# jianwang-mpi/GlobalEgoMocap

Hardware: AMD Instinct MI355X
Metric: optimised windows/sec (10-frame, 15-joint) (higher is better)
Workload: dtype f32

## Files before the change

### globalegomocap_amd/csrc/energy_device.h

```cpp
#pragma once
#include "gem_internal.h"

namespace gem {

__device__ __forceinline__ double wave_sum(double v) { return wave_sum_dpp(v); }
typedef float f32x4_t __attribute__((ext_vector_type(4)));

constexpr int MAXT = 16;
constexpr int MAXJ = GEM_MAX_JOINTS;
constexpr int ENERGY_SCRATCH = MAXT * MAXJ * 3;

template <bool BLOCK_SYNC>
__device__ __forceinline__ void energy_sync() {
    if (BLOCK_SYNC) {
        __syncthreads();
    } else {
        __builtin_amdgcn_fence(__ATOMIC_RELEASE, "workgroup");
        __builtin_amdgcn_wave_barrier();
        __builtin_amdgcn_fence(__ATOMIC_ACQUIRE, "workgroup");
    }
}

template <int NE, int NP>
struct EnergyPre {
    float x0[NE];
    float mb[NP];
    int par[NP];
    int key[NP];
    f32x4_t val[NP];
};
struct NoEnergyPre {};

template <int NT, int CN, typename F>
__device__ __forceinline__ void lane_pass(int lane, int n, F f) {
    if constexpr (CN > 0) {
#pragma unroll
        for (int it = 0; it < (CN + NT - 1) / NT; ++it) {
            const int e = lane + it * NT;
            if (e < CN) f(e, it);
        }
    } else {
        int it = 0;
        for (int e = lane; e < n; e += NT, ++it) f(e, it);
    }
}

template <int CT, int CJ>
__device__ __forceinline__ void energy_prefetch(const EnergyArgs& a, int b, int lane, EnergyPre<(CT * CJ * 3 + 63) / 64, (CT * CJ + 63) / 64>& pre) {
    constexpr int n = CT * CJ * 3, TJ = CT * CJ;
#pragma unroll
    for (int it = 0; it < (n + 63) / 64; ++it) {
        const int e = lane + it * 64;
        pre.x0[it] = e < n ? a.X0[(size_t)b * n + e] : 0.f;
    }
#pragma unroll
    for (int it = 0; it < (TJ + 63) / 64; ++it) {
        const int p = lane + it * 64;
        pre.mb[it] = 0.f; pre.par[it] = 0; pre.key[it] = -1; pre.val[it] = f32x4_t{0.f, 0.f, 0.f, 0.f};
        if (p < TJ) {
            const int j = p % CJ;
            pre.mb[it] = a.mean_bone[(size_t)b * CJ + j];
            pre.par[it] = a.parents[j];
            if (a.tex_key && a.wr != 0.f) {
                const size_t ci = (size_t)b * TJ + p;
                pre.key[it] = a.tex_key[ci];
                pre.val[it] = *reinterpret_cast<const f32x4_t*>(a.tex_val + ci * 4);
            }
        }
    }
}

struct FisheyeUV { float zz, nn, inv, rho, drho, ux, uy, u, v; };
__device__ __forceinline__ FisheyeUV fisheye_uv(const float* poly, int n_poly, float cx, float cy, float x, float y, float z) {
    FisheyeUV q;
    q.zz = -z;
    q.nn = sqrtf(x * x + y * y);
    q.inv = 1.f / q.nn;
    const float theta = atanf(q.zz / q.nn);
    float rho = poly[0], drho = 0.f, ti = 1.f;
    for (int i = 1; i < n_poly; ++i) {
        drho += (float)i * poly[i] * ti;
        ti *= theta;
        rho += ti * poly[i];
    }
    q.rho = rho; q.drho = drho;
    q.ux = x * q.inv; q.uy = y * q.inv;
    q.u = q.ux * rho + cx; q.v = q.uy * rho + cy;
    return q;
}

struct HeatTap { float fx, fy; bool in, xl, xr, yt, yb; int xa, xb, ya, yc; };
__device__ __forceinline__ HeatTap heat_tap(float u, float v, int H, int W) {
    HeatTap k;
    const float gxn = ((u - 128.f) - 512.f) / 512.f, gyn = (v - 512.f) / 512.f;
    const float ix = ((gxn + 1.f) / 2.f) * (float)(W - 1);
    const float iy = ((gyn + 1.f) / 2.f) * (float)(H - 1);
    const float fx0 = floorf(ix), fy0 = floorf(iy);
    k.fx = ix - fx0; k.fy = iy - fy0;
    k.in = fx0 >= -1.f && fx0 < (float)W && fy0 >= -1.f && fy0 < (float)H;
    const int x0i = k.in ? (int)fx0 : 0, y0i = k.in ? (int)fy0 : 0;
    k.xl = k.in && x0i >= 0; k.xr = k.in && x0i + 1 < W; k.yt = y0i >= 0; k.yb = y0i + 1 < H;
    k.xa = x0i < 0 ? 0 : x0i; k.xb = x0i + 1 < W ? x0i + 1 : W - 1;
    k.ya = y0i < 0 ? 0 : y0i; k.yc = y0i + 1 < H ? y0i + 1 : H - 1;
    return k;
}

__device__ __forceinline__ float heat_bilinear(const HeatTap& k, float& nw, float& ne, float& sw, float& se) {
    nw = (k.yt && k.xl) ? nw : 0.f;
    ne = (k.yt && k.xr) ? ne : 0.f;
    sw = (k.yb && k.xl) ? sw : 0.f;
    se = (k.yb && k.xr) ? se : 0.f;
    const float gxw = 1.f - k.fx, gyw = 1.f - k.fy;
    return nw * gxw * gyw + ne * k.fx * gyw + sw * gxw * k.fy + se * k.fx * k.fy;
}

template <bool BLOCK_SYNC, int NT = 64, int CT = 0, int CJ = 0, bool XS_IS_SRC = false, typename Pre = NoEnergyPre>
__device__ __forceinline__ void energy_window(const EnergyArgs& a, int b, int lane, const float* xsrc, int ldx, float* xs,
                                              float* gs, float* bs, float* as, float* gdst, int ldg, int gcols,
                                              uint16_t* gdst_b = nullptr, const float* x0_w = nullptr, const float* mb_w = nullptr,
                                              const int* par_w = nullptr, const int* ch_w = nullptr, const Pre* pre = nullptr) {
    static_assert(NT == 64 || BLOCK_SYNC, "more than one wavefront per window needs workgroup barriers");
    static_assert((CT > 0) == (CJ > 0), "give both compile-time dimensions or none");
    constexpr bool HAS_PRE = !__is_same(Pre, NoEnergyPre);
    static_assert(!HAS_PRE || (NT == 64 && CT > 0), "prefetched inputs are per lane of ONE wavefront with compile-time dimensions");
    const int T = CT ? CT : a.T, J = CJ ? CJ : a.J, JC = J * 3, n = T * JC;
    constexpr int CN = CT * CJ * 3, CP = CT * CJ;
    const float* x0 = x0_w ? x0_w : a.X0 + (size_t)b * n;
    const float* mbone = mb_w ? mb_w : a.mean_bone + (size_t)b * J;
    const int* parents = par_w ? par_w : a.parents;
    const int* children = ch_w ? ch_w : a.children;

    double e3d = 0, esm = 0, ebone = 0, evae = 0, erep = 0;
    lane_pass<NT, CN>(lane, n, [&](int e, int it) {
        const int t = e / JC, c = e - t * JC;
        const float x = xsrc[t * ldx + c];
        if (!XS_IS_SRC) xs[e] = x;
        float x0v;
        if constexpr (HAS_PRE) x0v = pre->x0[it]; else x0v = x0[e];
        const float d = x - x0v;
        e3d += (double)(d * d);
        evae += (double)(x * x);
        gs[e] = 2.f * a.w3d * d + 2.f * a.wv * x;
    });
    energy_sync<BLOCK_SYNC>();
    lane_pass<NT, CN>(lane, n, [&](int e, int) {
        const int t = e / JC;
        float acc = 0.f;
        if (t >= 1 && t <= T - 2) {
            acc = xs[e - JC] - 2.f * xs[e] + xs[e + JC];
            esm += (double)(acc * acc);
        }
        as[e] = acc;
    });
    lane_pass<NT, CP>(lane, T * J, [&](int p, int it) {
        const int t = p / J, j = p - t * J;
        int par;
        float mbv;
        if constexpr (HAS_PRE) { par = pre->par[it]; mbv = pre->mb[it]; } else { par = parents[j]; mbv = mbone[j]; }
        const float* xj = xs + (t * J + j) * 3;
        const float* xp = xs + (t * J + par) * 3;
        const float bx = xj[0] - xp[0], by = xj[1] - xp[1], bz = xj[2] - xp[2];
        const float len = sqrtf(bx * bx + by * by + bz * bz);
        const float diff = len - mbv;
        ebone += (double)(diff * diff);
        const float coef = len > 0.f ? 2.f * a.wb * diff / len : 0.f;
        float* o = bs + (t * J + j) * 3;
        o[0] = coef * bx; o[1] = coef * by; o[2] = coef * bz;
    });
    energy_sync<BLOCK_SYNC>();
    lane_pass<NT, CN>(lane, n, [&](int e, int) {
        const int t = e / JC;
        float g = gs[e];
        const float w2 = 2.f * a.ws;
        if (t >= 1 && t <= T - 2) g -= 2.f * w2 * as[e];
        if (t >= 2) g += w2 * as[e - JC];
        if (t <= T - 3) g += w2 * as[e + JC];
        gs[e] = g;
    });
    energy_sync<BLOCK_SYNC>();
    lane_pass<NT, CP>(lane, T * J, [&](int p, int it) {
        const int t = p / J, j = p - t * J;
        float gx = bs[p * 3 + 0], gy = bs[p * 3 + 1], gz = bs[p * 3 + 2];
        const int* ch = children + j * MAXJ;
        for (int q = 0; q < MAXJ && ch[q] >= 0; ++q) {
            const float* o = bs + (t * J + ch[q]) * 3;
            gx -= o[0]; gy -= o[1]; gz -= o[2];
        }
        if (a.wr != 0.f) {
            const float x = xs[p * 3 + 0], y = xs[p * 3 + 1], z = xs[p * 3 + 2];
            const FisheyeUV q = fisheye_uv(a.poly, a.n_poly, a.cx, a.cy, x, y, z);
            const float zz = q.zz, nn = q.nn, inv = q.inv, rho = q.rho, drho = q.drho, ux = q.ux, uy = q.uy;
            if (nn == 0.f) erep = __builtin_nan("");
            const HeatTap k = heat_tap(q.u, q.v, a.H, a.W);
            const float fx = k.fx, fy = k.fy;
            const bool in = k.in;
            const int xa = k.xa, xb = k.xb, ya = k.ya, yc = k.yc;
            const float* hm = a.heat + ((size_t)(a.frame0[b] + t) * a.H * a.W) * J + j;
            float nw, ne, sw, se;
            const int key = in ? (ya * a.W + xa) | ((yc * a.W + xb) << 16) : -1;
            const size_t ci = (size_t)b * (T * J) + p;
            bool hit = false;
            if (a.tex_key && in) {
                if constexpr (HAS_PRE) {
                    hit = pre->key[it] == key;
                    if (hit) { nw = pre->val[it][0]; ne = pre->val[it][1]; sw = pre->val[it][2]; se = pre->val[it][3]; }
                } else {
                    hit = a.tex_key[ci] == key;
                    if (hit) {
                        const f32x4_t c = *reinterpret_cast<const f32x4_t*>(a.tex_val + ci * 4);
                        nw = c[0]; ne = c[1]; sw = c[2]; se = c[3];
                    }
                }
            }
            if (!hit) {
                nw = hm[((size_t)ya * a.W + xa) * J];
                ne = hm[((size_t)ya * a.W + xb) * J];
                sw = hm[((size_t)yc * a.W + xa) * J];
                se = hm[((size_t)yc * a.W + xb) * J];
                if (a.tex_key && in) {
                    a.tex_key[ci] = key;
                    *reinterpret_cast<f32x4_t*>(a.tex_val + ci * 4) = f32x4_t{nw, ne, sw, se};
                }
            }
            const float val = heat_bilinear(k, nw, ne, sw, se);
            const float gxw = 1.f - fx, gyw = 1.f - fy;
            erep -= (double)val;
            const float dix = (ne - nw) * gyw + (se - sw) * fy;
            const float diy = (sw - nw) * gxw + (se - ne) * fx;
            const float gu = -a.wr * dix * ((float)(a.W - 1) / 1024.f);
            const float gv = -a.wr * diy * ((float)(a.H - 1) / 1024.f);
            const float r2 = nn * nn + zz * zz;
            const float dth_dn = -zz / r2, dth_dz = -nn / r2;
            const float i3 = inv * inv * inv;
            const float dudx = rho * (inv - x * x * i3) + ux * drho * dth_dn * ux;
            const float dudy = rho * (-x * y * i3) + ux * drho * dth_dn * uy;
            const float dudz = ux * drho * dth_dz;
            const float dvdx = rho * (-x * y * i3) + uy * drho * dth_dn * ux;
            const float dvdy = rho * (inv - y * y * i3) + uy * drho * dth_dn * uy;
            const float dvdz = uy * drho * dth_dz;
            gx += gu * dudx + gv * dvdx;
            gy += gu * dudy + gv * dvdy;
            gz += gu * dudz + gv * dvdz;
        }
        gs[p * 3 + 0] += gx; gs[p * 3 + 1] += gy; gs[p * 3 + 2] += gz;
    });
    energy_sync<BLOCK_SYNC>();
    if (CT > 0 && gcols == 64) {
        lane_pass<NT, CT * 64>(lane, T * 64, [&](int i, int) {
            const int t = i >> 6, c = i & 63;
            const float v = c < JC ? gs[t * JC + c] : 0.f;
            if (gdst_b) gdst_b[t * ldg + c] = (uint16_t)(__builtin_bit_cast(unsigned int, (float)(__bf16)v) >> 16);
            else gdst[t * ldg + c] = v;
        });
    } else {
        for (int i = lane; i < T * gcols; i += NT) {
            const int t = i / gcols, c = i - t * gcols;
            const float v = c < JC ? gs[t * JC + c] : 0.f;
            if (gdst_b) gdst_b[t * ldg + c] = (uint16_t)(__builtin_bit_cast(unsigned int, (float)(__bf16)v) >> 16);
            else gdst[t * ldg + c] = v;
        }
    }
    e3d = wave_sum(e3d); esm = wave_sum(esm); ebone = wave_sum(ebone); evae = wave_sum(evae); erep = wave_sum(erep);
    if (NT > 64) {
        double* red = reinterpret_cast<double*>(as);
        const int wv = lane >> 6;
        if ((lane & 63) == 0) { red[wv * 5 + 0] = e3d; red[wv * 5 + 1] = esm; red[wv * 5 + 2] = ebone; red[wv * 5 + 3] = evae; red[wv * 5 + 4] = erep; }
        __syncthreads();
        if (lane == 0) {
            e3d = esm = ebone = evae = erep = 0.0;
            for (int w = 0; w < NT / 64; ++w) {
                e3d += red[w * 5 + 0]; esm += red[w * 5 + 1]; ebone += red[w * 5 + 2]; evae += red[w * 5 + 3]; erep += red[w * 5 + 4];
            }
        }
    }
    if (lane == 0) {
        if (a.parts) {
            double* p = a.parts + (size_t)b * 5;
            p[0] = e3d; p[1] = esm; p[2] = ebone; p[3] = evae; p[4] = erep;
        }
        a.f[b] = a.dw3d * e3d + a.dws * esm + a.dwb * ebone + a.dwv * evae + a.dwr * erep;
    }
}

}
```

### globalegomocap_amd/csrc/gem_internal.h

```cpp
#pragma once
#if defined(__HIP_DEVICE_COMPILE__) && !defined(GEM_NO_PACKED_FP32)
#error "compile with: -Xclang -target-feature -Xclang -packed-fp32-ops -DGEM_NO_PACKED_FP32 (__graft_entry__.NO_PACKED_FP32)"
#endif

#include <hip/hip_runtime.h>
#include <stdint.h>
#include <atomic>
#include <set>
#include <string>
#include <vector>

#include "../../include/gem_hip.h"

namespace gem {

constexpr int PAD = 64;
constexpr float LEAKY_SLOPE = 0.01f;
constexpr double BN_EPS = 1e-5;
constexpr int MAX_HIST = 128;
constexpr int MAXJ_ERR = GEM_MAX_JOINTS;
constexpr int N_LOG = 1 << 16;
constexpr int TRACE_ROUNDS = 64;

inline int pad64(int x) { return (x + PAD - 1) / PAD * PAD; }
// ... 263 lines not shown
    if (s.dyn_W > 0) {
        const DynSplit d = dyn_split(*s.m_dev, 64, s.CT, s.dyn_W, s.n_tiles, s.ldc);
        nslab = d.SK;
        stride = d.slab;
    }
}
bool rows_can_fuse_compaction(const gem_handle* h, const Layer& L, int lda, int ldc, int B, bool slabs);
int launch_splitk_reduce(gem_handle* h, int epi, int nslab, size_t slab, const float* bias, const float* aux, float* C, int M, int N,
                         int ldc, const int* m_dev, hipStream_t s, int dyn_W = 0, int n_tiles = 0);
int launch_gemm_bf16(gem_handle* h, const Layer& L, int epi, int nprod, const float* A, int lda, const float* aux, float* Cout,
                     int ldc, int M, int T, hipStream_t s, const GemmOpts& o);

enum Narrow {
    NARROW_BATCHED = 0,
    NARROW_TAIL_F32 = 1,
    NARROW_TAIL_BF16 = 2
};
struct Route {
    int precision = 0;
    Narrow narrow = NARROW_BATCHED;
    bool front = false;
    int tail_wgs = 0;
    int tail_cap = 0;
    Repack repack = REPACK_KERNEL;
};
enum Call { CALL_DECODE = 0, CALL_EVALUATE = 1, CALL_ROUNDS = 2 };
Route plan_route(const gem_handle* h, int stage, int B, Call call);

struct EnergyArgs;
int evaluate_bf16(gem_handle* h, const Route& rt, int stage, int B, const EnergyArgs& ea, hipStream_t s, bool forward_only, const RoundSet* rs,
                  SlabSrc* grad);
int gemm_bf16a(gem_handle* h, const Layer& L, int epi, const uint16_t* A, int lda, const uint16_t* aux, void* C, bool out_bf16,
               int ldc, int M, hipStream_t s, int family, bool allow_split, const GemmOpts& o = GemmOpts());
int make_layer_images(std::vector<void*>& owner, Layer* L, int taps, int N, int K, const float* w, const float* bias);
int launch_f32_to_bf16(const float* src, uint16_t* dst, size_t n, hipStream_t s);
int launch_f32_split_bf16(const float* src, uint16_t* hi, uint16_t* lo, size_t n, hipStream_t s);

int launch_pack_pose(const float* src, float* dst, int rows, int C, hipStream_t s);
int launch_unpack_pose(const float* src, float* dst, int rows, int C, hipStream_t s);
int launch_reparam(const float* mulv, const float* eps, float* mu, float* logvar, float* z, float* z2, int B, int D, int Dp,
                   hipStream_t s);
int launch_pad_latent(const float* z, float* zp, int B, int D, int Dp, hipStream_t s);
int launch_unpad_latent(const float* zp, float* z, int B, int D, int Dp, hipStream_t s);

struct EnergyArgs {
    const float* Xp;
    const float* X0;
    const float* heat;
    const int32_t* frame0;
    const float* mean_bone;
    float* dXp;
    uint16_t* dXp_b;
    double* f;
    double* parts;
    float w3d, ws, wb, wv, wr;
    double dw3d, dws, dwb, dwv, dwr;
    int T, J, H, W, n_poly;
    float poly[GEM_MAX_POLY];
    float cx, cy;
    const int* parents;
    const int* children;
    int* tex_key;
    float* tex_val;
    const int* n_dev;
    const int* perm;
};
int launch_energy(gem_handle* h, const EnergyArgs& a, int B, hipStream_t s);

constexpr int TAIL_MAX_LAYERS = 6;
struct TailLayerDev { const float* w4; const float* bias; int K, N; };
struct TailArgs {
    int n, B, G, forward_only, escr, mask_first;
    int waves, rows;
    int maxnt;
    SlabSrc in_slab;
    const float* in_bias;
    int in_bias_ld;
    long long* dbg_ts;
    TailLayerDev fwd[TAIL_MAX_LAYERS], bwd[TAIL_MAX_LAYERS];
    const float* a_in;
    float* g_out;
    uint16_t* g_out_b;
    float* Xp;
    int off_act[TAIL_MAX_LAYERS + 1], ld_act[TAIL_MAX_LAYERS + 1], off_g[2], ld_g, off_red, off_escr, off_zero, off_pre;
    EnergyArgs e;
};
size_t plan_tail(const std::vector<Layer>& dec, int start, int T, int J, TailArgs* out, bool shared = false);
void fill_tail_args(const gem_handle* h, const StageNet& net, const Route& rt, int B, bool forward_only, const SlabSrc& in_slab,
                    const EnergyArgs& ea, const RoundSet* rs, TailArgs* ta);
size_t plan_tail_for(const gem_handle* h, const std::vector<Layer>& dec, int start, int wgs, TailArgs* out);

constexpr int TB_MAX_LAYERS = 6;
struct TailB16Layer { int K, N; const float* bias; };
struct TailB16Args {
    int n, B, G, nrt, forward_only, mask_first;
    SlabSrc in_slab;
    const float* in_bias;
    int in_bias_ld;
    const uint16_t* a_in_b;
    uint16_t* g_out_b;
    float* Xp;
    long long* dbg_ts;
    const uint16_t* wstream;
    int steps_f, steps_total;
    TailB16Layer fwd[TB_MAX_LAYERS], bwd[TB_MAX_LAYERS];
    int off_act[TB_MAX_LAYERS + 1], ld_act[TB_MAX_LAYERS + 1];
    int off_mask[TB_MAX_LAYERS], ld_mask[TB_MAX_LAYERS];
    int off_x, escr, off_mb, off_zero, off_tab;
    int off_bwin, off_epair;
    EnergyArgs e;
};
size_t plan_tail_bf16(const std::vector<Layer>& dec, int start, int T, int J, TailB16Args* out, int nrt = 5);
int tail_bf16_row_tiles(const gem_handle* h, int B, int T);
int build_tail_bf16_stream(gem_handle* h, StageNet& net);
int launch_tail_bf16(gem_handle* h, const TailB16Args& a, size_t lds_bytes, hipStream_t s, const RoundSet* rs = nullptr);
int launch_tail(gem_handle* h, const TailArgs& a, size_t lds_bytes, hipStream_t s, const RoundSet* rs = nullptr);
int tail_cap_workgroups(const gem_handle* h, const std::vector<Layer>& dec, int start);
int launch_mean_bone(gem_handle* h, const float* pose, int n_frames, float* out, hipStream_t s);
int launch_gather_windows(const float* frames, const int32_t* frame0, float* out, int B, int T, int JC, hipStream_t s);
int launch_relative_global(const float* local, const double* cams, const int32_t* frame0, float* rel, int B, int T, int J,
                           hipStream_t s);
int launch_to_global(const float* rel, const double* cams, const int32_t* frame0, double* out, int B, int T, int J,
                     hipStream_t s);

int launch_errors(gem_handle* h, const double* est, const double* mid, const double* opt, const double* gt, int F,
                  const double* bone_mm, double* frame_out, double* out, hipStream_t s, int n_seq);
int launch_merge(const double* win, double* tmp, double* out, int n_chunks, int wpc, int T, int JC, int overlap, int smooth,
                 hipStream_t s);
size_t errors_frame_lds_bytes(int J);
void drop_graphs(gem_handle* h);
int post_scratch(gem_handle* h, size_t elems);
int launch_lift(gem_handle* h, const float* heat, const double* depth, int F, const double* poly, int n_poly, int up, int pad_x,
                int pad_y, double* out64, float* out32, hipStream_t s);

int launch_lbfgs_init(gem_handle* h, int B, hipStream_t s);
int launch_lbfgs_advance(gem_handle* h, int B, const gem_lbfgs_opts& o, const RoundSet& rs, const SlabSrc& grad, hipStream_t s);
int launch_lbfgs_stats(gem_handle* h, int B, gem_window_stats* out, hipStream_t s);
int launch_compact(gem_handle* h, const RoundSet& rs, int B, int force_all, hipStream_t s, int zero_after = 0);
int launch_lbfgs_debug_read(gem_handle* h, int B, gem_lbfgs_debug_state* out, float* x, float* d, float* trial, hipStream_t s);


}
```

### globalegomocap_amd/csrc/tail.hip

```cpp
#include <algorithm>

#include "energy_device.h"

namespace gem {

typedef float f32x16 __attribute__((ext_vector_type(16)));
typedef float f32x4 __attribute__((ext_vector_type(4)));

__device__ __forceinline__ float bf16_round(float x) {
    const __bf16 b = (__bf16)x;
    return (float)b;
}

constexpr int TAIL_WAVES = 8;
constexpr int TAIL_THREADS = TAIL_WAVES * 64;
constexpr int TAIL_WAVES_SHARED = 4;

constexpr int TAIL_ROWS = 16;

#ifndef TAIL_PREFETCH_BLOCKS
#define TAIL_PREFETCH_BLOCKS 1
#endif
#ifndef TAIL_RING_DEPTH
#define TAIL_RING_DEPTH 2
#endif
#ifndef TAIL_PREFETCH_EARLY
#define TAIL_PREFETCH_EARLY 1
#endif
template <int W, int MAXNT>
struct TailSched {
    static constexpr bool DEEP = W == TAIL_WAVES && MAXNT <= 2;
    static constexpr int P = DEEP ? TAIL_PREFETCH_BLOCKS : 1;
    static constexpr int D = DEEP ? TAIL_RING_DEPTH : 2;
    static constexpr int NTP = DEEP ? MAXNT : 1;
    static constexpr int PW = P < D - 1 ? P : D - 1;
    static constexpr bool EARLY = DEEP && TAIL_PREFETCH_EARLY;
    static_assert(P >= 1 && D >= 2 && D <= 4, "ring of two to four register sets");
};
template <int W, int MAXNT>
struct TailPre {
    f32x4 b[TailSched<W, MAXNT>::P][4];
    f32x4 bx[TailSched<W, MAXNT>::NTP > 1 ? TailSched<W, MAXNT>::NTP - 1 : 1][TailSched<W, MAXNT>::PW][4];
    float bias[TailSched<W, MAXNT>::NTP];
};

template <int W, int MAXNT>
__device__ __forceinline__ void tail_prefetch(const TailLayerDev L, TailPre<W, MAXNT>& dst) {
    using S = TailSched<W, MAXNT>;
    const int lane = threadIdx.x & 63, wave = __builtin_amdgcn_readfirstlane(threadIdx.x >> 6);
    const int c = lane & 15, q = lane >> 4;
    const int n0 = wave * 16;
    if (n0 >= L.N) return;
    const int nblk = 3 * (L.K / 64);
    const int nb = nblk <= S::P ? nblk : S::PW;
    const char* p = reinterpret_cast<const char*>(reinterpret_cast<const f32x4*>(L.w4) + n0);
    const unsigned vo = (unsigned)(q * L.N + c) * 16u;
#pragma unroll
    for (int i = 0; i < S::NTP; ++i) {
        if (n0 + 16 * W * i < L.N) {
#pragma unroll
            for (int s = 0; s < (i == 0 ? S::P : S::PW); ++s) {
                if (s < nb) {
#pragma unroll
                    for (int g = 0; g < 4; ++g) {
                        const f32x4 v = *reinterpret_cast<const f32x4*>(p + (((size_t)16 * s + 4 * g) * L.N + 16 * W * i) * 16 + vo);
                        if (i == 0) dst.b[s][g] = v;
                        else dst.bx[i > 0 ? i - 1 : 0][s][g] = v;
                    }
                }
            }
            if constexpr (S::DEEP) dst.bias[i] = L.bias ? L.bias[n0 + 16 * W * i + c] : 0.f;
        }
    }
}

template <int W, int MAXNT, int NT, typename Epi>
__device__ __forceinline__ void tail_gemm_nt(const float* in, int ld_in, const float* zero_line, const TailLayerDev L,
                                             const TailLayerDev next, bool has_next, int T, int R, TailPre<W, MAXNT>& pre, Epi epi,
                                             int c0 = 0, bool use_pre = true) {
    using S = TailSched<W, MAXNT>;
    constexpr int P = S::P, D = S::D, NTP = S::NTP, PW = S::PW;
    const int tid = threadIdx.x, lane = tid & 63, wave = __builtin_amdgcn_readfirstlane(tid >> 6);
    const int fr = lane & 15, fq = lane >> 4;
// ... 67 lines not shown
        if (use_pre) {
#pragma unroll
            for (int s = 0; s < P; ++s) {
                if (s < PW || whole) {
#pragma unroll
                    for (int g = 0; g < 4; ++g) asm volatile("" : "+v"(pre.b[s][g]));
                }
            }
#pragma unroll
            for (int i = 1; i < (NT < NTP ? NT : NTP); ++i)
#pragma unroll
                for (int s = 0; s < PW; ++s)
#pragma unroll
                    for (int g = 0; g < 4; ++g) asm volatile("" : "+v"(pre.bx[i - 1][s][g]));
        }
        if (has_next) tail_prefetch<W, MAXNT>(next, pre_next);
    }
    TAIL_LOAD_A(0, a[0]);
    if (whole) {
        if constexpr (P >= 3 && NT == 1) {
            static_assert(P == 3, "a layer has at least three blocks: K = 64, three taps");
#pragma unroll
            for (int t = 0; t < P; ++t) TAIL_STEP(t, t, false, (&pre.b[t]));
        }
    } else {
#pragma unroll
        for (int s = 0; s < D - 1; ++s)
#pragma unroll
            for (int i = 0; i < NT; ++i) {
                if (s < PW && i < NTP && use_pre) {
#pragma unroll
                    for (int g = 0; g < 4; ++g) b[s][i][g] = i == 0 ? pre.b[s][g] : pre.bx[i > 0 ? i - 1 : 0][s < PW ? s : 0][g];
                } else TAIL_LOAD_B1(s, b[s], i);
            }
        const int nl = nblk - (D - 1), ngrp = nl / D, r = nl - ngrp * D;
        for (int grp = 0; grp < ngrp; ++grp) {
#pragma unroll
            for (int j = 0; j < D; ++j) TAIL_STEP(grp * D + j, j, true, b[j]);
        }
        const int blk0 = ngrp * D;
#pragma unroll
        for (int rr = 0; rr < D; ++rr) {
            if (r != rr) continue;
#pragma unroll
            for (int t = 0; t < rr + D - 1; ++t) TAIL_STEP(blk0 + t, t, t < rr, b[t % D]);
        }
    }
    if constexpr (S::EARLY) pre = pre_next;
    else if (has_next) tail_prefetch<W, MAXNT>(next, pre);
#undef TAIL_STEP
#undef TAIL_INTERLEAVE
#undef TAIL_LOAD_A
#undef TAIL_LOAD_B
#undef TAIL_LOAD_B1
#undef TAIL_COMPUTE
#pragma unroll
    for (int i = 0; i < NT; ++i) epi(acc[i], 4 * fq, n0 + TS * i + fr, bv[i]);
}

template <int W, int MAXNT, typename Epi>
__device__ __forceinline__ void tail_gemm(const float* in, int ld_in, const float* zero_line, const TailLayerDev L,
                                          const TailLayerDev next, bool has_next, int T, int R, TailPre<W, MAXNT>& pre, Epi epi) {
    if constexpr (W == TAIL_WAVES_SHARED) {
        if (L.N > 32 * W) {
            tail_gemm_nt<W, MAXNT, 2>(in, ld_in, zero_line, L, next, false, T, R, pre, epi);
            tail_gemm_nt<W, MAXNT, 2>(in, ld_in, zero_line, L, next, has_next, T, R, pre, epi, 32 * W, false);
        } else if (L.N > 16 * W) tail_gemm_nt<W, MAXNT, 2>(in, ld_in, zero_line, L, next, has_next, T, R, pre, epi);
        else tail_gemm_nt<W, MAXNT, 1>(in, ld_in, zero_line, L, next, has_next, T, R, pre, epi);
    } else {
        if constexpr (MAXNT >= 4) {
            if (L.N > 32 * W) { tail_gemm_nt<W, MAXNT, 4>(in, ld_in, zero_line, L, next, has_next, T, R, pre, epi); return; }
        }
        if (L.N > 16 * W) tail_gemm_nt<W, MAXNT, 2>(in, ld_in, zero_line, L, next, has_next, T, R, pre, epi);
        else tail_gemm_nt<W, MAXNT, 1>(in, ld_in, zero_line, L, next, has_next, T, R, pre, epi);
    }
}

template <int MAXNT>
struct TailTiles {
template <int NL, int W>
static __global__ __launch_bounds__(64 * W, W == TAIL_WAVES_SHARED ? 3 : 2) void decoder_tail_kernel(TailArgs a) {
    constexpr int THREADS = 64 * W;
    constexpr bool TIGHT = W == TAIL_WAVES_SHARED;
    constexpr int STAGE_U = 2048 / THREADS;
    constexpr int PRE_E = TAIL_THREADS / THREADS;
    extern __shared__ __attribute__((aligned(16))) float lds[];
    const int tid = threadIdx.x, lane = tid & 63, wave = __builtin_amdgcn_readfirstlane(tid >> 6);
    const int T = a.e.T;
    int probe = 0;
#define TAIL_PROBE()                                                                                   \
    if (a.dbg_ts && blockIdx.x == 0 && tid == 0) {                                                     \
        a.dbg_ts[2 * probe] = clock64();                                                               \
        a.dbg_ts[2 * probe + 1] = wall_clock64();                                                      \
        ++probe;                                                                                       \
    }
    const int w0 = blockIdx.x * a.G;
    const int B = a.e.n_dev ? *a.e.n_dev : a.B;
    if (w0 >= B) return;
    const int nwin = min(a.G, B - w0);
    const int R = nwin * T;
    const size_t row0 = (size_t)w0 * T;

    {
        const int K0 = a.fwd[0].K, q4 = K0 / 4, n4 = (TIGHT ? a.rows : TAIL_ROWS) * q4;
        float* dst = lds + a.off_act[0];
        if (a.in_slab.base) {
            int nslab;
            size_t stride;
            slab_layout(a.in_slab, nslab, stride);
            for (int u = 0; u < STAGE_U; ++u) {
                const int i = tid + u * THREADS, r = i / q4, c = (i - r * q4) * 4;
                if (i >= n4) break;
                f32x4 v = {0.f, 0.f, 0.f, 0.f};
                if (r < R) {
                    const float* p = a.in_slab.base + (row0 + r) * K0 + c;
                    for (int z0 = 0; z0 < nslab; z0 += 8) {
                        f32x4 t[8];
#pragma unroll
                        for (int k = 0; k < 8; ++k) t[k] = *reinterpret_cast<const f32x4*>(p + (size_t)min(z0 + k, nslab - 1) * stride);
#pragma unroll
                        for (int k = 0; k < 8; ++k)
                            if (z0 + k < nslab) v += t[k];
                    }
                    v += *reinterpret_cast<const f32x4*>(a.in_bias + (r % T) * a.in_bias_ld + c);
#pragma unroll
                    for (int q = 0; q < 4; ++q) v[q] = v[q] > 0.f ? v[q] : v[q] * LEAKY_SLOPE;
                }
                *reinterpret_cast<f32x4*>(dst + r * a.ld_act[0] + c) = v;
            }
        } else {
            f32x4 v[STAGE_U];
#pragma unroll
            for (int u = 0; u < STAGE_U; ++u) {
                const int i = tid + u * THREADS, r = i / q4, c = (i - r * q4) * 4;
                v[u] = f32x4{0.f, 0.f, 0.f, 0.f};
                if (i < n4 && r < R) v[u] = *reinterpret_cast<const f32x4*>(a.a_in + (row0 + r) * K0 + c);
            }
#pragma unroll
            for (int u = 0; u < STAGE_U; ++u) {
                const int i = tid + u * THREADS, r = i / q4, c = (i - r * q4) * 4;
                if (i < n4) *reinterpret_cast<f32x4*>(dst + r * a.ld_act[0] + c) = v[u];
            }
        }
        if (tid < 64) lds[a.off_zero + tid] = 0.f;
    }
    float pre_x0[PRE_E], pre_mb = 0.f;
    int pre_par = 0, pre_ch[PRE_E];
#pragma unroll
    for (int k = 0; k < PRE_E; ++k) { pre_x0[k] = 0.f; pre_ch[k] = -1; }
    static_assert(MAXJ * MAXJ <= TAIL_THREADS && MAXJ <= 64, "the children table is parked by PRE_E passes of the workgroup");
    const bool pre_on = a.G == 1 && !a.forward_only && T * a.e.J * 3 <= TAIL_THREADS;
    if (pre_on) {
        const int J = a.e.J, n = T * J * 3, bw = a.e.perm ? a.e.perm[w0] : w0;
#pragma unroll
        for (int k = 0; k < PRE_E; ++k) {
            const int e = tid + k * THREADS;
            if (e < n) pre_x0[k] = a.e.X0[(size_t)bw * n + e];
            if (e < J * MAXJ) pre_ch[k] = a.e.children[e];
        }
        if (tid < J) { pre_mb = a.e.mean_bone[(size_t)bw * J + tid]; pre_par = a.e.parents[tid]; }
    }
    TAIL_PROBE();
    __syncthreads();
    TAIL_PROBE();

    TailPre<W, MAXNT> bpre;
    tail_prefetch<W, MAXNT>(a.fwd[0], bpre);
#pragma unroll
    for (int i = 0; i < NL; ++i) {
        const bool last = (i + 1 == NL);
        float* out = lds + a.off_act[i + 1];
        const int ldo = a.ld_act[i + 1];
        float* Xp = last ? a.Xp : nullptr;
        const TailLayerDev nxt = !last ? a.fwd[i + 1 < NL ? i + 1 : i] : a.bwd[NL - 1];
        tail_gemm<W, MAXNT>(lds + a.off_act[i], a.ld_act[i], lds + a.off_zero, a.fwd[i], nxt, !last || !a.forward_only, T, R, bpre,
                  [&](const f32x4& acc, int r0, int col, float bv) {
#pragma unroll
                      for (int e = 0; e < 4; ++e) {
                          float v = acc[e] + bv;
                          if (!last) v = v > 0.f ? v : v * LEAKY_SLOPE;
                          if (!TIGHT || r0 + e < a.rows) out[(r0 + e) * ldo + col] = v;
                          if (Xp && r0 + e < R) Xp[(row0 + r0 + e) * PAD + col] = v;
                      }
                  });
        if (i == 0 && pre_on) {
            const int J = a.e.J, n = T * J * 3;
            float* pre = lds + a.off_pre;
            int* prei = reinterpret_cast<int*>(pre + n + J);
#pragma unroll
            for (int k = 0; k < PRE_E; ++k) {
                const int e = tid + k * THREADS;
                if (e < n) pre[e] = pre_x0[k];
                if (e < J * MAXJ) prei[J + e] = pre_ch[k];
            }
            if (tid < J) { pre[n + tid] = pre_mb; prei[tid] = pre_par; }
        }
        __syncthreads();
        TAIL_PROBE();
    }
    if (a.forward_only) return;

    float* g_cur = lds + a.off_g[0];
    float* g_nxt = lds + a.off_g[1];
    if (a.G == 1) {
        float* scr = lds + a.off_escr;
        const int J = a.e.J, n = T * J * 3;
        const float* pre = lds + a.off_pre;
        const int* prei = reinterpret_cast<const int*>(pre + n + J);
        if (T == 10 && J == 15)
            energy_window<true, THREADS, 10, 15>(a.e, a.e.perm ? a.e.perm[w0] : w0, tid, lds + a.off_act[NL], a.ld_act[NL], scr,
                                                      scr + a.escr, scr + 2 * a.escr, scr + 3 * a.escr, g_cur, a.ld_g, a.fwd[NL - 1].N,
                                                      nullptr, pre_on ? pre : nullptr, pre_on ? pre + n : nullptr, pre_on ? prei : nullptr,
                                                      pre_on ? prei + J : nullptr);
        else
            energy_window<true, THREADS>(a.e, a.e.perm ? a.e.perm[w0] : w0, tid, lds + a.off_act[NL], a.ld_act[NL], scr,
                                              scr + a.escr, scr + 2 * a.escr, scr + 3 * a.escr, g_cur, a.ld_g, a.fwd[NL - 1].N,
                                              nullptr, pre_on ? pre : nullptr, pre_on ? pre + n : nullptr, pre_on ? prei : nullptr,
                                              pre_on ? prei + J : nullptr);
    } else if (wave < nwin) {
        float* scr = lds + a.off_escr + wave * 4 * a.escr;
        energy_window<false>(a.e, a.e.perm ? a.e.perm[w0 + wave] : w0 + wave, lane,
                             lds + a.off_act[NL] + wave * T * a.ld_act[NL], a.ld_act[NL], scr, scr + a.escr,
                             scr + 2 * a.escr, scr + 3 * a.escr, g_cur + wave * T * a.ld_g, a.ld_g, a.fwd[NL - 1].N);
    }
    __syncthreads();
    TAIL_PROBE();

#pragma unroll
    for (int i = NL - 1; i >= 0; --i) {
        const float* act = lds + a.off_act[i];
        const int lda = a.ld_act[i];
        const int ldg = a.ld_g;
        float* gout = a.g_out;
        uint16_t* gout_b = a.g_out_b;
        const int K0 = a.fwd[0].K;
        tail_gemm<W, MAXNT>(g_cur, a.ld_g, lds + a.off_zero, a.bwd[i], a.bwd[i > 0 ? i - 1 : 0], i > 0, T, R, bpre,
                  [&](const f32x4& acc, int r0, int col, float) {
#pragma unroll
                      for (int e = 0; e < 4; ++e) {
                          const int row = r0 + e;
                          const float v = (i > 0 || a.mask_first) ? acc[e] * (act[row * lda + col] > 0.f ? 1.f : LEAKY_SLOPE) : acc[e];
                          if (i > 0) { if (!TIGHT || row < a.rows) g_nxt[row * ldg + col] = v; }
                          else if (row < R) {
                              if (gout_b) gout_b[(row0 + row) * K0 + col] = (uint16_t)(__builtin_bit_cast(unsigned int, bf16_round(v)) >> 16);
                              else gout[(row0 + row) * K0 + col] = v;
                          }
                      }
                  });
        __syncthreads();
        TAIL_PROBE();
        float* t = g_cur; g_cur = g_nxt; g_nxt = t;
    }
#undef TAIL_PROBE
}
};

size_t plan_tail(const std::vector<Layer>& dec, int start, int T, int J, TailArgs* out, bool shared) {
    const int n = (int)dec.size() - start;
    if (start < 0 || n < 1 || n > TAIL_MAX_LAYERS || T > TAIL_ROWS) return 0;
    for (int i = start; i < (int)dec.size(); ++i) {
        const int K = dec[i].K, N = dec[i].N;
        auto ok = [](int v) { return v == 64 || v == 128 || v == 256 || v == 512; };
        if (!ok(K) || !ok(N)) return 0;
    }
    TailArgs a{};
    a.n = n;
    a.mask_first = start > 0;
    a.G = TAIL_ROWS / T;
    if (shared && a.G != 1) return 0;
    a.waves = shared ? TAIL_WAVES_SHARED : TAIL_WAVES;
    a.rows = shared ? a.G * T : TAIL_ROWS;
    int widest = 0;
    for (int i = start; i < (int)dec.size(); ++i) widest = std::max(widest, std::max(dec[i].K, dec[i].N));
    a.maxnt = !shared && widest > 32 * TAIL_WAVES ? 4 : 2;
    const int rows = a.rows;
    int off = 0, maxg = 0;
    for (int i = 0; i <= n; ++i) {
        const int width = i == 0 ? dec[start].K : dec[start + i - 1].N;
        a.off_act[i] = off;
        a.ld_act[i] = width + 4;
        off += rows * (width + 4);
        if (i >= 1 && width > maxg) maxg = width;
    }
    a.ld_g = maxg + 4;
    a.off_g[0] = off; off += rows * a.ld_g;
    a.off_g[1] = off; off += rows * a.ld_g;
    a.escr = (T * J * 3 + 3) / 4 * 4;
    a.off_red = off;
    a.off_escr = off;
    off += a.G * 4 * a.escr;
    a.off_zero = off;
    off += 64;
    a.off_pre = off;
    if (a.G == 1) off += (T * J * 3 + 2 * J + J * MAXJ + 3) / 4 * 4;
    if (out) *out = a;
    return (size_t)off * sizeof(float);
}

template <int NL, int W, int MAXNT>
static void launch_tail_as(gem_handle* h, const TailArgs& a, int wgs, size_t lds_bytes, hipStream_t s) {
    note_kernel(h, reinterpret_cast<const void*>(&TailTiles<MAXNT>::template decoder_tail_kernel<NL, W>));
    hipLaunchKernelGGL((TailTiles<MAXNT>::template decoder_tail_kernel<NL, W>), dim3(wgs), dim3(64 * W), lds_bytes, s, a);
}

template <int W, int MAXNT>
static int launch_tail_w(gem_handle* h, const TailArgs& a, int wgs, size_t lds_bytes, hipStream_t s) {
    switch (a.n) {
        case 1: launch_tail_as<1, W, MAXNT>(h, a, wgs, lds_bytes, s); break;
        case 2: launch_tail_as<2, W, MAXNT>(h, a, wgs, lds_bytes, s); break;
        case 3: launch_tail_as<3, W, MAXNT>(h, a, wgs, lds_bytes, s); break;
        case 4: launch_tail_as<4, W, MAXNT>(h, a, wgs, lds_bytes, s); break;
        case 5: launch_tail_as<5, W, MAXNT>(h, a, wgs, lds_bytes, s); break;
        case 6: launch_tail_as<6, W, MAXNT>(h, a, wgs, lds_bytes, s); break;
        default: set_error("launch_tail: unsupported number of fused layers"); return 1;
    }
    return 0;
}

static bool tail_can_share_cu(const std::vector<Layer>& dec, int start, int T, int J) {
    const size_t bytes = plan_tail(dec, start, T, J, nullptr, true);
    if (!bytes || 3 * bytes > 160 * 1024) return false;
    for (int i = start; i < (int)dec.size(); ++i)
        if (dec[i].N > 64 * TAIL_WAVES_SHARED || dec[i].K > 64 * TAIL_WAVES_SHARED) return false;
    return true;
}

size_t plan_tail_for(const gem_handle* h, const std::vector<Layer>& dec, int start, int wgs, TailArgs* out) {
    bool shared = wgs > h->n_cu && tail_can_share_cu(dec, start, h->T, h->J);
    if (const char* f = dev_env("GEM_TAIL_WAVES")) shared = atoi(f) == TAIL_WAVES_SHARED && tail_can_share_cu(dec, start, h->T, h->J);
    return plan_tail(dec, start, h->T, h->J, out, shared);
}

int tail_cap_workgroups(const gem_handle* h, const std::vector<Layer>& dec, int start) {
    if (const char* f = dev_env("GEM_TAIL_CAP")) return atoi(f) * h->n_cu;
    return (tail_can_share_cu(dec, start, h->T, h->J) ? 10 : 5) * h->n_cu;
}

int launch_tail(gem_handle* h, const TailArgs& a, size_t lds_bytes, hipStream_t s, const RoundSet* rs) {
    static PerDeviceOnce attr_once;
    if (attr_once.need(h->cfg.device)) {
        const void* ks[] = {reinterpret_cast<const void*>(&TailTiles<2>::decoder_tail_kernel<1, 8>), reinterpret_cast<const void*>(&TailTiles<2>::decoder_tail_kernel<2, 8>),
                            reinterpret_cast<const void*>(&TailTiles<2>::decoder_tail_kernel<3, 8>), reinterpret_cast<const void*>(&TailTiles<2>::decoder_tail_kernel<4, 8>),
                            reinterpret_cast<const void*>(&TailTiles<2>::decoder_tail_kernel<5, 8>), reinterpret_cast<const void*>(&TailTiles<2>::decoder_tail_kernel<6, 8>),
                            reinterpret_cast<const void*>(&TailTiles<4>::decoder_tail_kernel<1, 8>), reinterpret_cast<const void*>(&TailTiles<4>::decoder_tail_kernel<2, 8>),
                            reinterpret_cast<const void*>(&TailTiles<4>::decoder_tail_kernel<3, 8>), reinterpret_cast<const void*>(&TailTiles<4>::decoder_tail_kernel<4, 8>),
                            reinterpret_cast<const void*>(&TailTiles<4>::decoder_tail_kernel<5, 8>), reinterpret_cast<const void*>(&TailTiles<4>::decoder_tail_kernel<6, 8>),
                            reinterpret_cast<const void*>(&TailTiles<2>::decoder_tail_kernel<1, 4>), reinterpret_cast<const void*>(&TailTiles<2>::decoder_tail_kernel<2, 4>),
                            reinterpret_cast<const void*>(&TailTiles<2>::decoder_tail_kernel<3, 4>), reinterpret_cast<const void*>(&TailTiles<2>::decoder_tail_kernel<4, 4>),
                            reinterpret_cast<const void*>(&TailTiles<2>::decoder_tail_kernel<5, 4>), reinterpret_cast<const void*>(&TailTiles<2>::decoder_tail_kernel<6, 4>)};
        for (const void* k : ks) GEM_HIP(hipFuncSetAttribute(k, hipFuncAttributeMaxDynamicSharedMemorySize, 160 * 1024));
    }
    Profile::Rec rec;
    const bool prof = h->prof.on;
    if (prof) {
        GEM_HIP(hipEventCreate(&rec.a)); GEM_HIP(hipEventCreate(&rec.b));
        rec.family = 1;
        double per_window = 0.0;
        for (int i = 0; i < a.n; ++i) per_window += 2.0 * 3.0 * a.fwd[i].K * a.fwd[i].N * a.e.T;
        if (!a.forward_only) per_window *= 2.0;
        rec.flops = per_window * a.B;
        if (rs) { rec.log_idx = rs->log_idx; rec.flops_per_window = per_window; }
        GEM_HIP(hipEventRecord(rec.a, s));
    }
    const int wgs = (a.B + a.G - 1) / a.G;
    bool planned = (a.waves == TAIL_WAVES && (a.maxnt == 2 || a.maxnt == 4)) || (a.waves == TAIL_WAVES_SHARED && a.maxnt == 2);
    for (int i = 0; planned && i < a.n && i < TAIL_MAX_LAYERS; ++i)
        planned = std::max(a.fwd[i].N, a.bwd[i].N) <= (a.waves == TAIL_WAVES ? 16 * TAIL_WAVES * a.maxnt : 64 * TAIL_WAVES_SHARED);
    if (!planned) { set_error("launch_tail: the arguments do not come from plan_tail"); return 1; }
    const int err = a.waves == TAIL_WAVES_SHARED ? launch_tail_w<TAIL_WAVES_SHARED, 2>(h, a, wgs, lds_bytes, s)
                    : a.maxnt == 4           ? launch_tail_w<TAIL_WAVES, 4>(h, a, wgs, lds_bytes, s)
                                             : launch_tail_w<TAIL_WAVES, 2>(h, a, wgs, lds_bytes, s);
    if (err) return 1;
    GEM_HIP(hipGetLastError());
    if (prof) { GEM_HIP(hipEventRecord(rec.b, s)); h->prof.recs.push_back(rec); }
    commit_kernel_names(h, prof ? 1 : -1);
    return 0;
}
// ... 3 lines not shown
```

Before: 32430.

## Hoist input staging and prefetches early, park heatmap cache in LDS

Result: no change. 32410, median of 2 (-0.1%).

```diff
diff --git a/globalegomocap_amd/csrc/energy_device.h b/globalegomocap_amd/csrc/energy_device.h
--- a/globalegomocap_amd/csrc/energy_device.h
+++ b/globalegomocap_amd/csrc/energy_device.h
@@ -30,6 +30,14 @@
     f32x4_t val[NP];
 };
 struct NoEnergyPre {};
+
+#ifdef TAIL_PROBE_FINE
+__device__ long long energy_probe_ts[5];
+#define ENERGY_PROBE(cond_, slot_, var_)                                                               \
+    if (NT > 64 && blockIdx.x == 0 && (cond_)) { asm volatile("" : "+v"(var_)); probe_ts[slot_] = wall_clock64(); }
+#else
+#define ENERGY_PROBE(cond_, slot_, var_)
+#endif
 
 template <int NT, int CN, typename F>
 __device__ __forceinline__ void lane_pass(int lane, int n, F f) {
@@ -118,7 +126,8 @@
 __device__ __forceinline__ void energy_window(const EnergyArgs& a, int b, int lane, const float* xsrc, int ldx, float* xs,
                                               float* gs, float* bs, float* as, float* gdst, int ldg, int gcols,
                                               uint16_t* gdst_b = nullptr, const float* x0_w = nullptr, const float* mb_w = nullptr,
-                                              const int* par_w = nullptr, const int* ch_w = nullptr, const Pre* pre = nullptr) {
+                                              const int* par_w = nullptr, const int* ch_w = nullptr, const float* tex_w = nullptr,
+                                              const Pre* pre = nullptr) {
     static_assert(NT == 64 || BLOCK_SYNC, "more than one wavefront per window needs workgroup barriers");
     static_assert((CT > 0) == (CJ > 0), "give both compile-time dimensions or none");
     constexpr bool HAS_PRE = !__is_same(Pre, NoEnergyPre);
@@ -131,6 +140,9 @@
     const int* children = ch_w ? ch_w : a.children;
 
     double e3d = 0, esm = 0, ebone = 0, evae = 0, erep = 0;
+#ifdef TAIL_PROBE_FINE
+    long long probe_ts[5] = {};
+#endif
     lane_pass<NT, CN>(lane, n, [&](int e, int it) {
         const int t = e / JC, c = e - t * JC;
         const float x = xsrc[t * ldx + c];
@@ -181,6 +193,7 @@
     lane_pass<NT, CP>(lane, T * J, [&](int p, int it) {
         const int t = p / J, j = p - t * J;
         float gx = bs[p * 3 + 0], gy = bs[p * 3 + 1], gz = bs[p * 3 + 2];
+        ENERGY_PROBE(p == 0, 0, gx);
         const int* ch = children + j * MAXJ;
         for (int q = 0; q < MAXJ && ch[q] >= 0; ++q) {
             const float* o = bs + (t * J + ch[q]) * 3;
@@ -195,17 +208,29 @@
             const float fx = k.fx, fy = k.fy;
             const bool in = k.in;
             const int xa = k.xa, xb = k.xb, ya = k.ya, yc = k.yc;
-            const float* hm = a.heat + ((size_t)(a.frame0[b] + t) * a.H * a.W) * J + j;
+            const int* texi_w = reinterpret_cast<const int*>(tex_w) + 4 * T * J;
+            const float* hm = a.heat + ((size_t)((tex_w ? texi_w[T * J] : a.frame0[b]) + t) * a.H * a.W) * J + j;
             float nw, ne, sw, se;
-            const int key = in ? (ya * a.W + xa) | ((yc * a.W + xb) << 16) : -1;
+            int key = in ? (ya * a.W + xa) | ((yc * a.W + xb) << 16) : -1;
+            ENERGY_PROBE(p == 0, 1, key);
             const size_t ci = (size_t)b * (T * J) + p;
             bool hit = false;
             if (a.tex_key && in) {
                 if constexpr (HAS_PRE) {
                     hit = pre->key[it] == key;
                     if (hit) { nw = pre->val[it][0]; ne = pre->val[it][1]; sw = pre->val[it][2]; se = pre->val[it][3]; }
+                } else if (tex_w) {
+                    int cached = texi_w[p];
+                    ENERGY_PROBE(p == 0, 2, cached);
+                    hit = cached == key;
+                    if (hit) {
+                        const f32x4_t c = *reinterpret_cast<const f32x4_t*>(tex_w + 4 * p);
+                        nw = c[0]; ne = c[1]; sw = c[2]; se = c[3];
+                    }
                 } else {
-                    hit = a.tex_key[ci] == key;
+                    int cached = a.tex_key[ci];
+                    ENERGY_PROBE(p == 0, 2, cached);
+                    hit = cached == key;
                     if (hit) {
                         const f32x4_t c = *reinterpret_cast<const f32x4_t*>(a.tex_val + ci * 4);
                         nw = c[0]; ne = c[1]; sw = c[2]; se = c[3];
@@ -222,6 +247,7 @@
                     *reinterpret_cast<f32x4_t*>(a.tex_val + ci * 4) = f32x4_t{nw, ne, sw, se};
                 }
             }
+            ENERGY_PROBE(p == 0, 3, nw);
             const float val = heat_bilinear(k, nw, ne, sw, se);
             const float gxw = 1.f - fx, gyw = 1.f - fy;
             erep -= (double)val;
@@ -245,6 +271,12 @@
         gs[p * 3 + 0] += gx; gs[p * 3 + 1] += gy; gs[p * 3 + 2] += gz;
     });
     energy_sync<BLOCK_SYNC>();
+#ifdef TAIL_PROBE_FINE
+    if (NT > 64 && blockIdx.x == 0 && lane == 0) {
+        probe_ts[4] = wall_clock64();
+        for (int i = 0; i < 5; ++i) energy_probe_ts[i] = probe_ts[i];
+    }
+#endif
     if (CT > 0 && gcols == 64) {
         lane_pass<NT, CT * 64>(lane, T * 64, [&](int i, int) {
             const int t = i >> 6, c = i & 63;
diff --git a/globalegomocap_amd/csrc/gem_internal.h b/globalegomocap_amd/csrc/gem_internal.h
--- a/globalegomocap_amd/csrc/gem_internal.h
+++ b/globalegomocap_amd/csrc/gem_internal.h
@@ -369,7 +369,7 @@
     float* g_out;
     uint16_t* g_out_b;
     float* Xp;
-    int off_act[TAIL_MAX_LAYERS + 1], ld_act[TAIL_MAX_LAYERS + 1], off_g[2], ld_g, off_red, off_escr, off_zero, off_pre;
+    int off_act[TAIL_MAX_LAYERS + 1], ld_act[TAIL_MAX_LAYERS + 1], off_g[2], ld_g, off_red, off_escr, off_zero, off_pre, off_tex;
     EnergyArgs e;
 };
 size_t plan_tail(const std::vector<Layer>& dec, int start, int T, int J, TailArgs* out, bool shared = false);
diff --git a/globalegomocap_amd/csrc/tail.hip b/globalegomocap_amd/csrc/tail.hip
--- a/globalegomocap_amd/csrc/tail.hip
+++ b/globalegomocap_amd/csrc/tail.hip
@@ -1,4 +1,5 @@
 #include <algorithm>
+#include <type_traits>
 
 #include "energy_device.h"
 
@@ -232,7 +233,8 @@
 static __global__ __launch_bounds__(64 * W, W == TAIL_WAVES_SHARED ? 3 : 2) void decoder_tail_kernel(TailArgs a) {
     constexpr int THREADS = 64 * W;
     constexpr bool TIGHT = W == TAIL_WAVES_SHARED;
-    constexpr int STAGE_U = 2048 / THREADS;
+    constexpr bool PARK_TEX = true;
+    constexpr int STAGE_U = 4;
     constexpr int PRE_E = TAIL_THREADS / THREADS;
     extern __shared__ __attribute__((aligned(16))) float lds[];
     const int tid = threadIdx.x, lane = tid & 63, wave = __builtin_amdgcn_readfirstlane(tid >> 6);
@@ -244,64 +246,134 @@
         a.dbg_ts[2 * probe + 1] = wall_clock64();                                                      \
         ++probe;                                                                                       \
     }
+#ifdef TAIL_PROBE_FINE
+    long long held[14] = {};
+#define TAIL_PROBE_START(k_, regular_)                                                                 \
+    if (a.dbg_ts && blockIdx.x == 0 && tid == 0) { held[2 * (k_)] = clock64(); held[2 * (k_) + 1] = wall_clock64(); }
+#else
+#define TAIL_PROBE_START(k_, regular_)                                                                 \
+    if (regular_) TAIL_PROBE();
+#endif
+    TAIL_PROBE_START(0, false);
     const int w0 = blockIdx.x * a.G;
-    const int B = a.e.n_dev ? *a.e.n_dev : a.B;
+    const size_t row0 = (size_t)w0 * T;
+
+    int vzero = 0;
+    asm volatile("" : "+v"(vzero));
+    int Bv = 0, bwv = w0;
+    if (a.e.n_dev) Bv = a.e.n_dev[vzero];
+    const bool one_window = a.G == 1 && !a.forward_only;
+    if (one_window && a.e.perm) bwv = a.e.perm[w0 + vzero];
+    TailPre<W, MAXNT> bpre;
+    tail_prefetch<W, MAXNT>(a.fwd[0], bpre);
+    const int K0 = a.fwd[0].K, q4 = K0 / 4, qs = 31 - __builtin_clz(q4), rows_staged = TIGHT ? a.rows : TAIL_ROWS;
+    const int Rmax = min(a.G, a.B - w0) * T;
+    int sr[STAGE_U], sc[STAGE_U];
+#pragma unroll
+    for (int u = 0; u < STAGE_U; ++u) {
+        const int i = tid + u * THREADS;
+        sr[u] = i >> qs;
+        sc[u] = (i & (q4 - 1)) * 4;
+    }
+    f32x4 v[STAGE_U];
+    if (a.in_slab.base) {
+        f32x4 bias[STAGE_U];
+        const float inv_T = 1.f / (float)T;
+        const char* bias_base = reinterpret_cast<const char*>(a.in_bias);
+#pragma unroll
+        for (int u = 0; u < STAGE_U; ++u) {
+            const int r = sr[u], t = r - T * (int)(((float)r + 0.5f) * inv_T);
+            v[u] = bias[u] = f32x4{0.f, 0.f, 0.f, 0.f};
+            if (r < rows_staged && r < Rmax) bias[u] = *reinterpret_cast<const f32x4*>(bias_base + (unsigned)(t * a.in_bias_ld + sc[u]) * 4u);
+        }
+        int nslab;
+        size_t stride;
+        slab_layout(a.in_slab, nslab, stride);
+#ifdef TAIL_PROBE_FINE
+        bool first_group = true;
+#endif
+        const char* slab_base = reinterpret_cast<const char*>(a.in_slab.base + row0 * K0);
+        auto add_slabs = [&](auto ns, int z0) {
+            constexpr int NS = decltype(ns)::value;
+            f32x4 t[STAGE_U][NS];
+#pragma unroll
+            for (int u = 0; u < STAGE_U; ++u) {
+#pragma unroll
+                for (int k = 0; k < NS; ++k) t[u][k] = f32x4{0.f, 0.f, 0.f, 0.f};
+                if (sr[u] < rows_staged && sr[u] < Rmax) {
+                    const unsigned vo = (unsigned)(sr[u] * K0 + sc[u]) * 4u;
+#pragma unroll
+                    for (int k = 0; k < NS; ++k)
+                        t[u][k] = *reinterpret_cast<const f32x4*>(slab_base + (size_t)min(z0 + k, nslab - 1) * stride * sizeof(float) + vo);
+                }
+            }
+#ifdef TAIL_PROBE_FINE
+            if (first_group) {
+                TAIL_PROBE_START(1, false);
+                asm volatile("" : "+v"(Bv), "+v"(bwv));
+                TAIL_PROBE_START(2, false);
+                first_group = false;
+            }
+#endif
+#pragma unroll
+            for (int u = 0; u < STAGE_U; ++u)
+#pragma unroll
+                for (int k = 0; k < NS; ++k) asm volatile("" : "+v"(t[u][k]));
+#pragma unroll
+            for (int u = 0; u < STAGE_U; ++u)
+#pragma unroll
+                for (int k = 0; k < NS; ++k)
+                    if (z0 + k < nslab) v[u] += t[u][k];
+        };
+        if (nslab <= 2) add_slabs(std::integral_constant<int, 2>{}, 0);
+        else
+            for (int z0 = 0; z0 < nslab; z0 += 4) add_slabs(std::integral_constant<int, 4>{}, z0);
+#pragma unroll
+        for (int u = 0; u < STAGE_U; ++u) {
+            v[u] += bias[u];
+#pragma unroll
+            for (int q = 0; q < 4; ++q) v[u][q] = v[u][q] > 0.f ? v[u][q] : v[u][q] * LEAKY_SLOPE;
+        }
+    } else {
+        const char* in_base = reinterpret_cast<const char*>(a.a_in + row0 * K0);
+#pragma unroll
+        for (int u = 0; u < STAGE_U; ++u) {
+            v[u] = f32x4{0.f, 0.f, 0.f, 0.f};
+            if (sr[u] < rows_staged && sr[u] < Rmax) v[u] = *reinterpret_cast<const f32x4*>(in_base + (unsigned)(sr[u] * K0 + sc[u]) * 4u);
+        }
+#ifdef TAIL_PROBE_FINE
+        TAIL_PROBE_START(1, false);
+        asm volatile("" : "+v"(Bv), "+v"(bwv));
+        TAIL_PROBE_START(2, false);
+#endif
+    }
+    asm volatile("" : "+v"(Bv), "+v"(bwv));
+#pragma unroll
+    for (int u = 0; u < STAGE_U; ++u) asm volatile("" : "+v"(v[u]));
+    TAIL_PROBE_START(3, false);
+    const int B = a.e.n_dev ? __builtin_amdgcn_readfirstlane(Bv) : a.B;
     if (w0 >= B) return;
     const int nwin = min(a.G, B - w0);
     const int R = nwin * T;
-    const size_t row0 = (size_t)w0 * T;
-
     {
-        const int K0 = a.fwd[0].K, q4 = K0 / 4, n4 = (TIGHT ? a.rows : TAIL_ROWS) * q4;
         float* dst = lds + a.off_act[0];
-        if (a.in_slab.base) {
-            int nslab;
-            size_t stride;
-            slab_layout(a.in_slab, nslab, stride);
-            for (int u = 0; u < STAGE_U; ++u) {
-                const int i = tid + u * THREADS, r = i / q4, c = (i - r * q4) * 4;
-                if (i >= n4) break;
-                f32x4 v = {0.f, 0.f, 0.f, 0.f};
-                if (r < R) {
-                    const float* p = a.in_slab.base + (row0 + r) * K0 + c;
-                    for (int z0 = 0; z0 < nslab; z0 += 8) {
-                        f32x4 t[8];
-#pragma unroll
-                        for (int k = 0; k < 8; ++k) t[k] = *reinterpret_cast<const f32x4*>(p + (size_t)min(z0 + k, nslab - 1) * stride);
-#pragma unroll
-                        for (int k = 0; k < 8; ++k)
-                            if (z0 + k < nslab) v += t[k];
-                    }
-                    v += *reinterpret_cast<const f32x4*>(a.in_bias + (r % T) * a.in_bias_ld + c);
-#pragma unroll
-                    for (int q = 0; q < 4; ++q) v[q] = v[q] > 0.f ? v[q] : v[q] * LEAKY_SLOPE;
-                }
-                *reinterpret_cast<f32x4*>(dst + r * a.ld_act[0] + c) = v;
-            }
-        } else {
-            f32x4 v[STAGE_U];
-#pragma unroll
-            for (int u = 0; u < STAGE_U; ++u) {
-                const int i = tid + u * THREADS, r = i / q4, c = (i - r * q4) * 4;
-                v[u] = f32x4{0.f, 0.f, 0.f, 0.f};
-                if (i < n4 && r < R) v[u] = *reinterpret_cast<const f32x4*>(a.a_in + (row0 + r) * K0 + c);
-            }
-#pragma unroll
-            for (int u = 0; u < STAGE_U; ++u) {
-                const int i = tid + u * THREADS, r = i / q4, c = (i - r * q4) * 4;
-                if (i < n4) *reinterpret_cast<f32x4*>(dst + r * a.ld_act[0] + c) = v[u];
-            }
-        }
+#pragma unroll
+        for (int u = 0; u < STAGE_U; ++u)
+            if (sr[u] < rows_staged) *reinterpret_cast<f32x4*>(dst + sr[u] * a.ld_act[0] + sc[u]) = sr[u] < R ? v[u] : f32x4{0.f, 0.f, 0.f, 0.f};
         if (tid < 64) lds[a.off_zero + tid] = 0.f;
     }
+    const int bw = __builtin_amdgcn_readfirstlane(bwv);
     float pre_x0[PRE_E], pre_mb = 0.f;
     int pre_par = 0, pre_ch[PRE_E];
 #pragma unroll
     for (int k = 0; k < PRE_E; ++k) { pre_x0[k] = 0.f; pre_ch[k] = -1; }
     static_assert(MAXJ * MAXJ <= TAIL_THREADS && MAXJ <= 64, "the children table is parked by PRE_E passes of the workgroup");
-    const bool pre_on = a.G == 1 && !a.forward_only && T * a.e.J * 3 <= TAIL_THREADS;
+    const bool pre_on = one_window && T * a.e.J * 3 <= TAIL_THREADS;
+    const bool pre_tex = PARK_TEX && pre_on && a.e.tex_key && a.e.wr != 0.f;
+    int pre_key = -1, pre_f0 = 0;
+    f32x4 pre_val = {0.f, 0.f, 0.f, 0.f};
     if (pre_on) {
-        const int J = a.e.J, n = T * J * 3, bw = a.e.perm ? a.e.perm[w0] : w0;
+        const int J = a.e.J, n = T * J * 3;
 #pragma unroll
         for (int k = 0; k < PRE_E; ++k) {
             const int e = tid + k * THREADS;
@@ -309,13 +381,29 @@
             if (e < J * MAXJ) pre_ch[k] = a.e.children[e];
         }
         if (tid < J) { pre_mb = a.e.mean_bone[(size_t)bw * J + tid]; pre_par = a.e.parents[tid]; }
-    }
-    TAIL_PROBE();
+        if (pre_tex) {
+            if (tid < T * J) {
+                const size_t ci = (size_t)bw * (T * J) + tid;
+                pre_key = a.e.tex_key[ci];
+                pre_val = *reinterpret_cast<const f32x4*>(a.e.tex_val + ci * 4);
+            }
+            if (tid == 0) pre_f0 = a.e.frame0[bw];
+        }
+    }
+    TAIL_PROBE_START(4, true);
     __syncthreads();
-    TAIL_PROBE();
-
-    TailPre<W, MAXNT> bpre;
-    tail_prefetch<W, MAXNT>(a.fwd[0], bpre);
+    TAIL_PROBE_START(5, true);
+#ifdef TAIL_PROBE_FINE
+#pragma unroll
+    for (int g = 0; g < 4; ++g) asm volatile("" : "+v"(bpre.b[0][g]));
+    TAIL_PROBE_START(6, false);
+    if (a.dbg_ts && blockIdx.x == 0 && tid == 0) {
+#pragma unroll
+        for (int k = 0; k < 14; ++k) a.dbg_ts[k] = held[k];
+        probe = 7;
+    }
+#endif
+
 #pragma unroll
     for (int i = 0; i < NL; ++i) {
         const bool last = (i + 1 == NL);
@@ -344,6 +432,12 @@
                 if (e < J * MAXJ) prei[J + e] = pre_ch[k];
             }
             if (tid < J) { pre[n + tid] = pre_mb; prei[tid] = pre_par; }
+            if (pre_tex) {
+                float* tex = lds + a.off_tex;
+                int* texi = reinterpret_cast<int*>(tex + 4 * T * J);
+                if (tid < T * J) { *reinterpret_cast<f32x4*>(tex + 4 * tid) = pre_val; texi[tid] = pre_key; }
+                if (tid == 0) texi[T * J] = pre_f0;
+            }
         }
         __syncthreads();
         TAIL_PROBE();
@@ -357,16 +451,17 @@
         const int J = a.e.J, n = T * J * 3;
         const float* pre = lds + a.off_pre;
         const int* prei = reinterpret_cast<const int*>(pre + n + J);
+        const float* tex = pre_tex ? lds + a.off_tex : nullptr;
         if (T == 10 && J == 15)
-            energy_window<true, THREADS, 10, 15>(a.e, a.e.perm ? a.e.perm[w0] : w0, tid, lds + a.off_act[NL], a.ld_act[NL], scr,
+            energy_window<true, THREADS, 10, 15>(a.e, bw, tid, lds + a.off_act[NL], a.ld_act[NL], scr,
                                                       scr + a.escr, scr + 2 * a.escr, scr + 3 * a.escr, g_cur, a.ld_g, a.fwd[NL - 1].N,
                                                       nullptr, pre_on ? pre : nullptr, pre_on ? pre + n : nullptr, pre_on ? prei : nullptr,
-                                                      pre_on ? prei + J : nullptr);
+                                                      pre_on ? prei + J : nullptr, tex);
         else
-            energy_window<true, THREADS>(a.e, a.e.perm ? a.e.perm[w0] : w0, tid, lds + a.off_act[NL], a.ld_act[NL], scr,
+            energy_window<true, THREADS>(a.e, bw, tid, lds + a.off_act[NL], a.ld_act[NL], scr,
                                               scr + a.escr, scr + 2 * a.escr, scr + 3 * a.escr, g_cur, a.ld_g, a.fwd[NL - 1].N,
                                               nullptr, pre_on ? pre : nullptr, pre_on ? pre + n : nullptr, pre_on ? prei : nullptr,
-                                              pre_on ? prei + J : nullptr);
+                                              pre_on ? prei + J : nullptr, tex);
     } else if (wave < nwin) {
         float* scr = lds + a.off_escr + wave * 4 * a.escr;
         energy_window<false>(a.e, a.e.perm ? a.e.perm[w0 + wave] : w0 + wave, lane,
@@ -397,10 +492,11 @@
                           }
                       }
                   });
-        __syncthreads();
+        if (i > 0 || a.dbg_ts) __syncthreads();
         TAIL_PROBE();
         float* t = g_cur; g_cur = g_nxt; g_nxt = t;
     }
+#undef TAIL_PROBE_START
 #undef TAIL_PROBE
 }
 };
@@ -443,6 +539,8 @@
     off += 64;
     a.off_pre = off;
     if (a.G == 1) off += (T * J * 3 + 2 * J + J * MAXJ + 3) / 4 * 4;
+    a.off_tex = a.off_g[0];
+    if (a.G == 1 && 2 * rows * a.ld_g < 5 * T * J + 1) return 0;
     if (out) *out = a;
     return (size_t)off * sizeof(float);
 }
```
